# google/deepconsensus

Measured on AMD Instinct MI355X. Metric: zmw_per_sec, higher is better.
Workload: dtype bf16; 1 GPU; global_batch=16384, seq_len=100, windows_per_zmw=150, parallelism=dp1, native_kernels=True, hipgraph=True

## Files before the change

### deepconsensus_amd/models/runner.py

```python
from __future__ import annotations

import copy
import math
from typing import List, Optional, Tuple

import torch

from deepconsensus_amd import ops as dc_ops
from deepconsensus_amd.calibration.calibration import (
    parse_calibration_string,
)
from deepconsensus_amd.models.config import Params
from deepconsensus_amd.models.model import (
    EncoderOnlyLearnedValuesTransformer,
    get_model,
)
from deepconsensus_amd.utils import constants
from deepconsensus_amd.utils import trace


def build_gather_tables(model: EncoderOnlyLearnedValuesTransformer):
    (bi, pwi, ipi, sti, ci, bqi, sni) = model.indices

    def scaled(emb):
# ... 144 lines not shown
            self._prepare_native(model)

    def _prepare_native(self, model) -> None:
        dev, bf16 = self.device, torch.bfloat16
        tf, rs, rv, cc, ce = build_gather_tables(model)
        self.table_flat = tf.to(dev)
        self.row_shift = rs.to(dev)
        self.row_vocab = rv.to(dev)
        self.chunk_cnt = cc.to(dev)
        self.chunk_entries = ce.to(dev)
        self.win = model.params.get("attn_win_size")
        self.num_heads = model.params["num_heads"]
        self.cond_wt = (
            model.condenser.weight.detach().t().contiguous().to(bf16).to(dev)
        )
        self.pos = (
            model.pos_encoding.to(bf16).to(dev)
            if model.add_pos_encoding
            else None
        )
        import os as _os

        self.cond_img = None
        self.pos_f32 = None
        cw = model.condenser.weight.detach()
        if fused_condense_enabled(
            cw.shape[1], _os.environ.get("DC_FUSED_CONDENSE")
        ):
            self.cond_img = build_condense_image(cw).to(dev)
            if model.add_pos_encoding:
                self.pos_f32 = (
                    model.pos_encoding.detach().float().contiguous().to(dev)
                )
        self.rezero_fast = all(
            l.attn_wrap.rezero and l.ffn_wrap.rezero for l in model.layers
        ) and self.win is not None
        if self.rezero_fast:
            self.layer_w = []
            for l in model.layers:
                wq = l.attn.q_proj.weight.detach()
                wk = l.attn.k_proj.weight.detach()
                wv = l.attn.v_proj.weight.detach()
                wqkv_t = (
                    torch.cat([wq, wk, wv], 0).t().contiguous().to(bf16).to(dev)
                )
                self.layer_w.append(
                    dict(
                        wqkv_t=wqkv_t,
                        wout_t=l.attn.out_proj.weight.detach()
                        .t().contiguous().to(bf16).to(dev),
                        w1_t=l.ffn.filter_layer.weight.detach()
                        .t().contiguous().to(bf16).to(dev),
                        b1=l.ffn.filter_layer.bias.detach().to(bf16).to(dev),
                        w2_t=l.ffn.output_layer.weight.detach()
                        .t().contiguous().to(bf16).to(dev),
                        b2=l.ffn.output_layer.bias.detach().to(bf16).to(dev),
                        alpha_attn=float(l.attn_wrap.alpha.detach()),
                        alpha_ffn=float(l.ffn_wrap.alpha.detach()),
                    )
                )
            for lw in self.layer_w:
                lw["wout_t_a"] = lw["wout_t"] * lw["alpha_attn"]
                lw["w2_t_a"] = lw["w2_t"] * lw["alpha_ffn"]
                lw["b2_a"] = lw["b2"] * lw["alpha_ffn"]
            import os as _os

# ... 40 lines not shown
                    lw["w1_v2"] = w1v2.to(bf16).contiguous().to(dev)
            self._addmm_act = hasattr(torch, "_addmm_activation")
            if self._addmm_act:
                try:
                    torch._addmm_activation(
                        torch.zeros(4, device=dev, dtype=bf16),
                        torch.zeros(2, 4, device=dev, dtype=bf16),
                        torch.zeros(4, 4, device=dev, dtype=bf16),
                    )
                except Exception:
                    self._addmm_act = False
        else:
            layers = copy.deepcopy(model.layers).to(bf16)
            for m in layers.modules():
                if isinstance(m, torch.nn.LayerNorm):
                    m.float()
            self.layers_bf16 = layers.to(dev)
        self.ln_gamma = model.output_norm.weight.detach().float().to(dev)
        self.ln_beta = model.output_norm.bias.detach().float().to(dev)
        self.w_head = model.fc1.weight.detach().float().contiguous().to(dev)
        self.b_head = model.fc1.bias.detach().float().to(dev)

    def _attn(self, qkv: torch.Tensor) -> torch.Tensor:
        b, l, w = qkv.shape
        d = w // (3 * self.num_heads)
        if d == 140 and 32 <= l <= 104 and 1 <= self.win <= 12:
            return self.ext.banded_attn_mfma(
                qkv, self.num_heads, self.win, d ** -0.5
            )
        return self.ext.banded_attn(qkv, self.num_heads, self.win)

    @torch.no_grad()
    def encode_native(self, rows: torch.Tensor) -> torch.Tensor:
        with trace.range("K2_embed_gather"):
            emb = self.ext.embed_gather(
                rows.contiguous(), self.table_flat, self.row_shift,
                self.row_vocab, self.chunk_cnt, self.chunk_entries,
            )
        b, l, _ = emb.shape
        if self.cond_img is not None:
            with trace.range("K3_condenser"):
                h = self.cond_wt.shape[1]
                pos = (
                    self.pos_f32
                    if self.pos_f32 is not None
                    else emb.new_empty(0, dtype=torch.float32)
                )
                x = self.ext.fused_condense(
                    emb.reshape(b * l, -1), self.cond_img, pos, h, l
                )
            x = x.view(b, l, -1)
        else:
            with trace.range("K3_condenser"):
                x = emb.reshape(b * l, -1) @ self.cond_wt
            x = x.view(b, l, -1)
            if self.pos is not None:
                x = x + self.pos[:l]
        if self.rezero_fast:
            h = x.shape[-1]
            flat = x.reshape(b * l, h)
            empty = flat.new_empty(0)
            for lw in self.layer_w:
                with trace.range("K5_qkv_proj"):
                    if self.ffn_fused_ok:
                        qkv = self.ext.fused_linear(
                            flat, lw["wqkv_pad"], empty, empty, 840,
                            False, 0.0
                        ).view(b, l, -1)
                    else:
                        qkv = (flat @ lw["wqkv_t"]).view(b, l, -1)
                with trace.range("K6_banded_attn"):
                    a = self._attn(qkv)
                if self.ffn_fused_ok:
                    with trace.range("K7_out_proj"):
                        flat = self.ext.fused_linear(
                            a.view(b * l, h), lw["wout_pad"], empty, flat,
                            280, False, lw["alpha_attn"],
                        )
                    with trace.range("K9_fused_ffn"):
                        if self.ffn_v5:
                            flat = self.ext.fused_ffn_v5(
                                flat, lw["w1_v2"], lw["w2_pad"],
                                lw["b2_f32"], lw["alpha_ffn"],
                            )
                        elif self.ffn_v3:
# ... 109 lines not shown
```

### deepconsensus_amd/ops/build.py

```python
from __future__ import annotations

import os
import shutil

_OPS_DIR = os.path.dirname(os.path.abspath(__file__))
_BUILD_DIR = os.path.join(_OPS_DIR, "_build")
_SRCS = [
    os.path.join(_OPS_DIR, "hip", "dc_kernels.hip"),
    os.path.join(_OPS_DIR, "hip", "banded_attn.hip"),
    os.path.join(_OPS_DIR, "hip", "banded_attn_mfma.hip"),
    os.path.join(_OPS_DIR, "hip", "embed_gather.hip"),
    os.path.join(_OPS_DIR, "hip", "fused_ffn.hip"),
    os.path.join(_OPS_DIR, "hip", "alignment_dp.hip"),
    os.path.join(_OPS_DIR, "hip", "fused_linear.hip"),
    os.path.join(_OPS_DIR, "hip", "fused_ffn_glds.hip"),
    os.path.join(_OPS_DIR, "hip", "fused_ffn_v3.hip"),
    os.path.join(_OPS_DIR, "hip", "embed_grad.hip"),
    os.path.join(_OPS_DIR, "hip", "alignment_metric.hip"),
    os.path.join(_OPS_DIR, "hip", "ffn_ablate.hip"),
    os.path.join(_OPS_DIR, "hip", "banded_attn_train.hip"),
    os.path.join(_OPS_DIR, "hip", "banded_attn_bwd_mfma.hip"),
    os.path.join(_OPS_DIR, "hip", "fused_condense.hip"),
    os.path.join(_OPS_DIR, "hip", "ffn_train.hip"),
    os.path.join(_OPS_DIR, "hip", "resid_dropout.hip"),
    os.path.join(_OPS_DIR, "hip", "stitch_compact.hip"),
    os.path.join(_OPS_DIR, "hip", "window_featurize.hip"),
    os.path.join(_OPS_DIR, "hip", "passthrough_fill.hip"),
    os.path.join(_OPS_DIR, "hip", "subread_space.hip"),
    os.path.join(_OPS_DIR, "hip", "fused_ffn_v5.hip"),
    os.path.join(_OPS_DIR, "hip", "alignment_calib.hip"),
]
EXT_NAME = "dc_hip_kernels"


_SPACING_SRC = os.path.join(
    os.path.dirname(_OPS_DIR), "preprocess", "_spacing_cpp.cpp"
)


def build_spacing(verbose: bool = False):
    os.makedirs(_BUILD_DIR, exist_ok=True)
    from torch.utils.cpp_extension import load

    return load(
        name="_spacing",
        sources=[_SPACING_SRC],
        build_directory=_BUILD_DIR,
        extra_cflags=["-O3"],
        verbose=verbose,
    )


def build(verbose: bool = False):
    os.environ.setdefault("PYTORCH_ROCM_ARCH", "gfx950")
    os.makedirs(_BUILD_DIR, exist_ok=True)
# ... 40 lines not shown
```

### deepconsensus_amd/ops/hip/dc_kernels.hip

```cpp

#ifndef DC_SAN_MAIN
#include <torch/extension.h>
#include <ATen/hip/HIPContext.h>
#endif
#include <hip/hip_runtime.h>
#include <hip/hip_bf16.h>

#define DC_CHECK(x, msg) TORCH_CHECK(x, msg)

using bf16 = __hip_bfloat16;

namespace {

template <typename T>
__global__ __launch_bounds__(256) void fused_ln_head_qv_kernel(
    const T* __restrict__ x, const float* __restrict__ gamma,
    const float* __restrict__ beta, const float* __restrict__ w_head,
    const float* __restrict__ b_head, uint8_t* __restrict__ bases_out,
    uint8_t* __restrict__ quals_out, float* __restrict__ probs_out,
    int N, int H, float cal_threshold, float cal_w, float cal_b,
    float max_qual) {
  const int wave_in_block = threadIdx.x >> 6;
  const int lane = threadIdx.x & 63;
  for (int n = blockIdx.x * 4 + wave_in_block; n < N; n += gridDim.x * 4) {
  const T* xi = x + (size_t)n * H;

  float sum = 0.f;
  float xv[8];
  int nd = 0;
  for (int d = lane; d < H; d += 64, ++nd) {
    float v;
    if constexpr (std::is_same_v<T, bf16>) v = __bfloat162float(xi[d]);
    else v = xi[d];
    xv[nd] = v;
    sum += v;
  }
#pragma unroll
  for (int off = 32; off > 0; off >>= 1) sum += __shfl_xor(sum, off, 64);
  const float mean = sum / H;
  float sq = 0.f;
  nd = 0;
  for (int d = lane; d < H; d += 64, ++nd) {
    const float dv = xv[nd] - mean;
    sq += dv * dv;
  }
#pragma unroll
  for (int off = 32; off > 0; off >>= 1) sq += __shfl_xor(sq, off, 64);
  const float var = sq / H;
  const float rstd = rsqrtf(var + 1e-6f);

  float logit[5];
#pragma unroll
  for (int k = 0; k < 5; ++k) logit[k] = 0.f;
  nd = 0;
  for (int d = lane; d < H; d += 64, ++nd) {
    const float normed = (xv[nd] - mean) * rstd * gamma[d] + beta[d];
#pragma unroll
    for (int k = 0; k < 5; ++k) logit[k] += normed * w_head[k * H + d];
  }
#pragma unroll
  for (int off = 32; off > 0; off >>= 1) {
#pragma unroll
    for (int k = 0; k < 5; ++k) logit[k] += __shfl_xor(logit[k], off, 64);
  }

  if (lane == 0) {
    float mx = -1e30f;
#pragma unroll
    for (int k = 0; k < 5; ++k) {
      logit[k] += b_head[k];
      mx = fmaxf(mx, logit[k]);
    }
    float denom = 0.f;
    float ex[5];
#pragma unroll
    for (int k = 0; k < 5; ++k) {
      ex[k] = __expf(logit[k] - mx);
      denom += ex[k];
    }
    int arg = 0;
    float pmax = 0.f;
#pragma unroll
    for (int k = 0; k < 5; ++k) {
      const float p = ex[k] / denom;
      if (probs_out != nullptr) probs_out[(size_t)n * 5 + k] = p;
      if (p > pmax) { pmax = p; arg = k; }
    }
    float ep = 1.f - pmax;
    float q = (ep <= 0.f) ? 1e9f : -10.f * log10f(ep);
    if (cal_threshold == 0.f || q > cal_threshold) q = q * cal_w + cal_b;
    q = fminf(q, max_qual);
// ... 2 lines not shown
    bases_out[n] = (uint8_t)arg;
    quals_out[n] = (uint8_t)q;
  }
  }
}

}

#ifndef DC_SAN_MAIN

std::vector<at::Tensor> fused_ln_head_qv(
    at::Tensor x, at::Tensor gamma, at::Tensor beta, at::Tensor w_head,
    at::Tensor b_head, double cal_threshold, double cal_w, double cal_b,
    double max_qual, bool want_probs) {
  DC_CHECK(x.is_cuda() && x.dim() >= 2, "x must be a device matrix");
  auto xc = x.contiguous();
  const int H = xc.size(-1);
  const int N = xc.numel() / H;
  DC_CHECK(H <= 512, "H must be <= 512");
  auto opts = xc.options();
  auto bases = at::empty({N}, opts.dtype(at::kByte));
  auto quals = at::empty({N}, opts.dtype(at::kByte));
  at::Tensor probs;
  float* probs_ptr = nullptr;
  if (want_probs) {
    probs = at::empty({N, 5}, opts.dtype(at::kFloat));
    probs_ptr = probs.data_ptr<float>();
  }
  dim3 grid(std::min((N + 3) / 4, 2048));
  dim3 block(256);
  hipStream_t stream = at::hip::getCurrentHIPStream();
  auto gc = gamma.contiguous(), bc = beta.contiguous();
  auto wc = w_head.contiguous(), bhc = b_head.contiguous();
  if (xc.dtype() == at::kBFloat16) {
    hipLaunchKernelGGL(fused_ln_head_qv_kernel<bf16>, grid, block, 0, stream,
                       reinterpret_cast<bf16*>(xc.data_ptr()),
                       gc.data_ptr<float>(), bc.data_ptr<float>(),
                       wc.data_ptr<float>(), bhc.data_ptr<float>(),
                       bases.data_ptr<uint8_t>(), quals.data_ptr<uint8_t>(),
                       probs_ptr, N, H, (float)cal_threshold, (float)cal_w,
                       (float)cal_b, (float)max_qual);
  } else {
    DC_CHECK(xc.dtype() == at::kFloat, "x must be bf16 or fp32");
    hipLaunchKernelGGL(fused_ln_head_qv_kernel<float>, grid, block, 0, stream,
                       xc.data_ptr<float>(), gc.data_ptr<float>(),
                       bc.data_ptr<float>(), wc.data_ptr<float>(),
                       bhc.data_ptr<float>(), bases.data_ptr<uint8_t>(),
                       quals.data_ptr<uint8_t>(), probs_ptr, N, H,
                       (float)cal_threshold, (float)cal_w, (float)cal_b,
                       (float)max_qual);
  }
  if (want_probs) return {bases, quals, probs};
  return {bases, quals};
}

at::Tensor banded_attn(at::Tensor qkv, int64_t H, int64_t win);
at::Tensor banded_attn_mfma(at::Tensor qkv, int64_t H, int64_t win,
                            double scale);
at::Tensor embed_gather(at::Tensor rows, at::Tensor table_flat,
                        at::Tensor row_shift, at::Tensor row_vocab,
                        at::Tensor chunk_cnt, at::Tensor chunk_entries);
at::Tensor fused_ffn(at::Tensor x, at::Tensor w1, at::Tensor b1,
                     at::Tensor w2, at::Tensor b2, double alpha);
at::Tensor fused_ffn_v2(at::Tensor x, at::Tensor w1, at::Tensor w2,
                        at::Tensor b2, double alpha);
at::Tensor fused_ffn_v3(at::Tensor x, at::Tensor w1, at::Tensor w2,
                        at::Tensor b2, double alpha);
at::Tensor fused_ffn_v5(at::Tensor x, at::Tensor w1, at::Tensor w2,
                        at::Tensor b2, double alpha, int64_t max_blocks);
void embed_grad(at::Tensor rows, at::Tensor grad_out, at::Tensor row_shift,
                at::Tensor row_vocab, at::Tensor row_tbase,
                at::Tensor row_width, at::Tensor row_col,
                at::Tensor row_scale, at::Tensor grad_tables);
at::Tensor fused_linear(at::Tensor x, at::Tensor w, at::Tensor bias,
                        at::Tensor resid, int64_t n_out, bool relu,
                        double alpha);
std::vector<at::Tensor> alignment_dp_fwd(at::Tensor subs, at::Tensor ins,
                                         at::Tensor seq_lens, double del_cost,
                                         double reg, int64_t width);
std::vector<at::Tensor> alignment_dp_bwd(at::Tensor grad_out,
                                         at::Tensor weights,
                                         at::Tensor seq_lens, int64_t m,
                                         int64_t n, int64_t width);
std::vector<at::Tensor> alignment_metric_counts(
    at::Tensor yt, at::Tensor yp, at::Tensor yt_len, at::Tensor yp_len,
    double ms, double mp, double go, double ge);
std::vector<at::Tensor> alignment_calib(
    at::Tensor label, at::Tensor bases, at::Tensor quals,
    double ms, double mp, double go, double ge);
at::Tensor ffn_ablate(at::Tensor x, at::Tensor w1, at::Tensor w2,
                      at::Tensor b2, double alpha, int64_t mode);
std::vector<at::Tensor> banded_attn_train_fwd(
    at::Tensor q, at::Tensor k, at::Tensor v, at::Tensor mask,
    int64_t win, double p_drop);
std::vector<at::Tensor> banded_attn_train_bwd(
    at::Tensor q, at::Tensor k, at::Tensor v, at::Tensor p,
    at::Tensor mask, at::Tensor dout, int64_t win, double p_drop);
std::vector<at::Tensor> banded_attn_mfma_train_fwd(
    at::Tensor qkv, int64_t H, int64_t win, double scale,
    at::Tensor drop_mask, double p_drop);
at::Tensor banded_attn_train_bwd2(
    at::Tensor qkv, at::Tensor p, at::Tensor mask, at::Tensor dout,
    int64_t H, int64_t win, double p_drop);
at::Tensor banded_attn_bwd_mfma(
    at::Tensor qkv, at::Tensor p, at::Tensor mask, at::Tensor dout,
    int64_t H, int64_t win, double p_drop);
at::Tensor fused_condense(at::Tensor x, at::Tensor w, at::Tensor pos,
                          int64_t n_out, int64_t seq_len);
std::vector<at::Tensor> ffn_train_fwd(at::Tensor x, at::Tensor w1,
                                      at::Tensor w2, at::Tensor b2,
                                      double p_drop, int64_t seed);
std::vector<at::Tensor> ffn_train_dgrad(at::Tensor dy, at::Tensor hd,
                                        at::Tensor w2t, at::Tensor w1t,
                                        double p_drop);
std::vector<at::Tensor> ffn_train_dgrad_nomask(at::Tensor dy, at::Tensor hd,
                                               at::Tensor w2t,
                                               at::Tensor w1t,
                                               double p_drop);
at::Tensor resid_drop_fwd(at::Tensor x, at::Tensor y, double alpha,
                          double p_drop, int64_t seed);
std::vector<at::Tensor> resid_drop_bwd(at::Tensor dout, at::Tensor y,
                                       double alpha, double p_drop,
                                       int64_t seed);
std::vector<at::Tensor> stitch_compact(at::Tensor bases, at::Tensor quals,
                                       at::Tensor seg_off,
                                       at::Tensor seg_len);
int64_t stitch_compact_into(at::Tensor bases, at::Tensor quals,
                            at::Tensor seg_off, at::Tensor seg_len,
                            at::Tensor seq_out, at::Tensor qual_out,
                            at::Tensor seg_kept, at::Tensor out_off);
at::Tensor window_featurize(at::Tensor sub, at::Tensor ccs,
                            at::Tensor ccs_bq, at::Tensor zmw_tab,
                            at::Tensor win_tab, int64_t R, int64_t L,
                            int64_t max_passes, bool use_ccs_bq);
void window_featurize_into(at::Tensor sub, at::Tensor ccs,
                           at::Tensor ccs_bq, at::Tensor zmw_tab,
                           at::Tensor win_tab, at::Tensor out,
                           int64_t max_passes, bool use_ccs_bq);
void passthrough_fill_into(at::Tensor ccs, at::Tensor ccs_q,
                           at::Tensor zmw_tab, at::Tensor pt_tab,
                           at::Tensor qual_lut, at::Tensor bases_out,
                           at::Tensor quals_out);
void subread_space_into(at::Tensor src, at::Tensor ins_max,
                        at::Tensor sp_tab, at::Tensor read_tab,
                        at::Tensor zmw_tab, at::Tensor col_ref,
                        at::Tensor sub, at::Tensor ccs, at::Tensor ccs_q,
                        at::Tensor ccs_bq, bool use_ccs_bq);
int64_t subread_space_tile();

PYBIND11_MODULE(TORCH_EXTENSION_NAME, m) {
  m.def("subread_space_into", &subread_space_into,
        "Device subread spacing: unspaced reads + ins_max -> caller-owned "
        "zero-filled sub / ccs / ccs_q / ccs_bq planes");
  m.def("subread_space_tile", &subread_space_tile,
        "Scan tile (elements) of subread_space_into");
  m.def("passthrough_fill_into", &passthrough_fill_into,
        "Device CCS passthrough: skipped windows of the packed planes -> "
        "caller-owned base-id and QV rows of the stitch buffer");
  m.def("window_featurize", &window_featurize,
        "Device window featurization: compact ZMW planes + window table "
        "-> int16 [N, R, L] model input");
  m.def("window_featurize_into", &window_featurize_into,
        "window_featurize into a caller-owned int16 [N, R, L] tensor");
  m.def("stitch_compact", &stitch_compact,
        "Device window stitching: segmented gap compaction -> (seq_out, "
        "qual_out, seg_kept, out_off)");
  m.def("stitch_compact_into", &stitch_compact_into,
        "stitch_compact into caller-owned output buffers; returns "
        "out_off[S]");
  m.def("fused_condense", &fused_condense,
        "Condenser GEMM [M,560]x[560,N] + fused position-encoding add "
        "(K3+K4)");
  m.def("ffn_train_fwd", &ffn_train_fwd,
        "Training FFN forward: relu + hash dropout in-register, returns "
        "(y, hd)");
  m.def("ffn_train_dgrad", &ffn_train_dgrad,
        "Training FFN dgrad: both transposed GEMMs fused, mask from hd>0, "
        "returns (dx, dh_pre)");
  m.def("ffn_train_dgrad_nomask", &ffn_train_dgrad_nomask,
        "Bisection probe: dgrad without the mask (dh == dy@W2^T)");
  m.def("resid_drop_fwd", &resid_drop_fwd,
        "Fused ReZero residual + hash-dropout forward");
  m.def("resid_drop_bwd", &resid_drop_bwd,
        "Fused residual-dropout backward: (dy, dalpha partials)");
  m.def("fused_ln_head_qv", &fused_ln_head_qv,
        "Fused final LayerNorm + head + softmax + QV (K10+K11+K12)");
  m.def("banded_attn", &banded_attn,
        "Banded multi-head self-attention forward (K5-K7 core, generic)");
  m.def("banded_attn_mfma", &banded_attn_mfma,
        "Banded MHA forward on MFMA (D=140, L<=104)");
  m.def("embed_gather", &embed_gather,
        "Subread-stack embedding gather (K2)");
  m.def("fused_ffn", &fused_ffn,
        "Fused FFN + ReZero residual (K8+K9), hidden tensor LDS-resident");
  m.def("fused_ffn_v2", &fused_ffn_v2,
        "Fused FFN v2: glds-pipelined weights, bias folded into W1");
  m.def("fused_ffn_v3", &fused_ffn_v3,
        "Fused FFN v3: 256-row tiles, register-resident h (swapped B1)");
  m.def("fused_ffn_v5", &fused_ffn_v5,
        "Fused FFN v5: v3 chunk loop in a persistent grid (continuous "
        "weight stream, direct x fragments, 16-B epilogue); max_blocks "
        "caps the grid, 0 = one block per CU",
        pybind11::arg("x"), pybind11::arg("w1"), pybind11::arg("w2"),
        pybind11::arg("b2"), pybind11::arg("alpha"),
        pybind11::arg("max_blocks") = 0);
// ... 33 lines not shown
```

### deepconsensus_amd/ops/hip/fused_condense.hip

```cpp

#ifndef DC_SAN_MAIN
#include <torch/extension.h>
#include <ATen/hip/HIPContext.h>
#endif
#include <hip/hip_runtime.h>
#include <hip/hip_bf16.h>

using bf16 = __hip_bfloat16;

namespace {

typedef __bf16 bf16x8 __attribute__((ext_vector_type(8)));
typedef float f32x16 __attribute__((ext_vector_type(16)));

constexpr int NC = 64;
constexpr int O_STRIDE = 72;

template <int K>
struct CondCfg {
  static constexpr int NG = (K + 15) / 16;
  static constexpr int WS = 16 * NG + 8;
  static constexpr bool HALF = (K % 16) == 8;
  static constexpr int NW = NG <= 36 ? 8 : 4;
  static constexpr int BM = 32 * NW;
  static constexpr int NT = 64 * NW;
  static constexpr int UNITS = NC * WS * 2 / 1024;
  static_assert(K % 8 == 0, "rows must stay 16-B aligned");
  static_assert((NC * WS * 2) % 1024 == 0, "chunk must be whole KiB units");
  static_assert((NC * WS + BM * O_STRIDE) * 2 <= 160 * 1024, "LDS budget");
};

__device__ __forceinline__ int lane_recompute() {
  int l;
  asm volatile(
      "v_mbcnt_lo_u32_b32 %0, -1, 0\n\t"
      "v_mbcnt_hi_u32_b32 %0, -1, %0"
      : "=v"(l));
  return l;
}

template <int K>
__global__ __launch_bounds__(CondCfg<K>::NT, 1) void fused_condense_kernel(
    const bf16* __restrict__ x, const bf16* __restrict__ w,
    const float* __restrict__ pos, bf16* __restrict__ out,
    int M, int N, int Npad, int L) {
  using C = CondCfg<K>;
  constexpr int NG = C::NG;
  constexpr int W_STRIDE = C::WS;
  constexpr int BM = C::BM;
  constexpr int NW = C::NW;
  constexpr int NT = C::NT;
  __shared__ __attribute__((aligned(16))) bf16 w_lds[NC * W_STRIDE];
  __shared__ __attribute__((aligned(16))) bf16 o_lds[BM * O_STRIDE];

  const int tid = threadIdx.x;
  const int wave = __builtin_amdgcn_readfirstlane(tid >> 6);
  const int m0 = blockIdx.x * BM;

  auto issue_w = [&](int chunk) {
    const int ln = lane_recompute();
    const bf16* src = w + (size_t)chunk * NC * W_STRIDE;
    constexpr int TRIPS = (C::UNITS + NW - 1) / NW;
    constexpr int UNROLL = NW == 8 ? TRIPS : 4;
#pragma unroll UNROLL
    for (int i = 0; i < TRIPS; ++i) {
      const int ck = wave + i * NW;
      if (ck < C::UNITS) {
        __builtin_amdgcn_global_load_lds(
            (const __attribute__((address_space(1))) unsigned*)(
                src + ck * 512 + ln * 8),
            (__attribute__((address_space(3))) unsigned*)(
                &w_lds[ck * 512]),
            16, 0, 0);
      }
    }
  };

  issue_w(0);

  bf16x8 af[NG];
  {
    const int ln = lane_recompute();
    const int row = m0 + 32 * wave + (ln & 31);
    constexpr int NFULL = C::HALF ? NG - 1 : NG;
    if (row < M) {
      const bf16* xr = x + (size_t)row * K + 8 * (ln >> 5);
#pragma unroll
      for (int s = 0; s < NFULL; ++s) {
        af[s] = *reinterpret_cast<const bf16x8*>(xr + 16 * s);
      }
    } else {
#pragma unroll
      for (int s = 0; s < NFULL; ++s) af[s] = bf16x8{};
    }
    if constexpr (C::HALF) {
      af[NG - 1] = bf16x8{};
      if (row < M && (ln >> 5) == 0) {
        af[NG - 1] = *reinterpret_cast<const bf16x8*>(
            x + (size_t)row * K + 16 * (NG - 1));
      }
    }
  }
  asm volatile("s_waitcnt vmcnt(0)" ::: "memory");
  __builtin_amdgcn_s_barrier();

  const int nchunk = Npad / NC;
  for (int chunk = 0; chunk < nchunk; ++chunk) {
    const int ln = lane_recompute();
    const int c = ln & 31;
    const int hi = ln >> 5;
#pragma unroll
    for (int ch = 0; ch < 2; ++ch) {
      const int colt = 32 * ch;
      const int ncol = chunk * NC + colt + c;
      f32x16 acc0 = {}, acc1 = {};
      __builtin_amdgcn_s_setprio(1);
#pragma unroll
      for (int s = 0; s < NG; s += 2) {
        const bf16x8 b0 = *reinterpret_cast<const bf16x8*>(
            &w_lds[(colt + c) * W_STRIDE + 16 * s + 8 * hi]);
        acc0 = __builtin_amdgcn_mfma_f32_32x32x16_bf16(af[s], b0, acc0,
                                                       0, 0, 0);
        if (s + 1 < NG) {
          const bf16x8 b1 = *reinterpret_cast<const bf16x8*>(
              &w_lds[(colt + c) * W_STRIDE + 16 * (s + 1) + 8 * hi]);
          acc1 = __builtin_amdgcn_mfma_f32_32x32x16_bf16(af[s + 1], b1,
                                                         acc1, 0, 0, 0);
        }
      }
      __builtin_amdgcn_s_setprio(0);
#pragma unroll
      for (int r = 0; r < 16; ++r) {
        const int row = (r & 3) + 8 * (r >> 2) + 4 * hi + 32 * wave;
        float v = acc0[r] + acc1[r];
        if (pos != nullptr && ncol < N && m0 + row < M) {
          v += pos[(size_t)((m0 + row) % L) * N + ncol];
        }
        o_lds[row * O_STRIDE + colt + c] = __float2bfloat16(v);
      }
    }
    __syncthreads();
    if (chunk + 1 < nchunk) issue_w(chunk + 1);

    const int n0 = chunk * NC;
    for (int idx = tid; idx < BM * (NC / 8); idx += NT) {
      const int row = idx / (NC / 8), c8 = idx % (NC / 8);
      if (m0 + row >= M) continue;
      const int col = n0 + 8 * c8;
      if (col >= N) continue;
      const bf16x8 v = *reinterpret_cast<const bf16x8*>(
          &o_lds[row * O_STRIDE + 8 * c8]);
      if (col + 8 <= N) {
        *reinterpret_cast<bf16x8*>(
            out + (size_t)(m0 + row) * N + col) = v;
      } else {
        const unsigned short* vs =
            reinterpret_cast<const unsigned short*>(&v);
        for (int j = 0; j < 8 && col + j < N; ++j) {
          reinterpret_cast<unsigned short*>(
              out)[(size_t)(m0 + row) * N + col + j] = vs[j];
        }
      }
    }
    if (chunk + 1 < nchunk) {
      asm volatile("s_waitcnt vmcnt(0) lgkmcnt(0)" ::: "memory");
    }
    __builtin_amdgcn_s_barrier();
  }
}

#define DC_CONDENSE_INST(K)                                       \
  template __global__ void fused_condense_kernel<K>(              \
      const bf16* __restrict__, const bf16* __restrict__,         \
      const float* __restrict__, bf16* __restrict__, int, int, int, int)
DC_CONDENSE_INST(560);
DC_CONDENSE_INST(568);
DC_CONDENSE_INST(872);
DC_CONDENSE_INST(880);
#undef DC_CONDENSE_INST

}

#ifndef DC_SAN_MAIN

namespace {

template <int K>
void launch_condense(const at::Tensor& xc, const at::Tensor& w,
                     const float* pos_ptr, at::Tensor& out, int M, int N,
                     int Npad, int L) {
  using C = CondCfg<K>;
  TORCH_CHECK(w.size(1) == C::WS, "fused_condense: width-", K,
              " input needs a weight image of row stride ", C::WS,
              ", got ", w.size(1));
  dim3 grid((M + C::BM - 1) / C::BM);
  dim3 block(C::NT);
  hipStream_t stream = at::hip::getCurrentHIPStream();
  hipLaunchKernelGGL(fused_condense_kernel<K>, grid, block, 0, stream,
                     reinterpret_cast<bf16*>(xc.data_ptr()),
                     reinterpret_cast<bf16*>(w.data_ptr()), pos_ptr,
                     reinterpret_cast<bf16*>(out.data_ptr()), M, N, Npad,
// ... 44 lines not shown
```

Before: 2471 ZMWs/sec.

## Fuse embedding gather into condenser GEMM and register-cache LN head params

Adds a fused kernel that gathers embedding rows directly into MFMA A-fragments inside the condenser GEMM, so the intermediate [M,K] embedding tensor is never written to or read back from global memory. The shared condense tile code moves into a header and both kernels use it. The LN+head kernel also keeps gamma, beta and the head weights in registers and prefetches the next row. The cost is more register pressure and scattered gathers inside the GEMM prologue.

```diff
diff --git a/deepconsensus_amd/models/runner.py b/deepconsensus_amd/models/runner.py
--- a/deepconsensus_amd/models/runner.py
+++ b/deepconsensus_amd/models/runner.py
@@ -200,6 +200,7 @@
                 self.pos_f32 = (
                     model.pos_encoding.detach().float().contiguous().to(dev)
                 )
+        self.fused_embed = _os.environ.get("DC_FUSED_EMBED") != "0"
         self.rezero_fast = all(
             l.attn_wrap.rezero and l.ffn_wrap.rezero for l in model.layers
         ) and self.win is not None
@@ -306,25 +307,35 @@
 
     @torch.no_grad()
     def encode_native(self, rows: torch.Tensor) -> torch.Tensor:
-        with trace.range("K2_embed_gather"):
-            emb = self.ext.embed_gather(
-                rows.contiguous(), self.table_flat, self.row_shift,
-                self.row_vocab, self.chunk_cnt, self.chunk_entries,
-            )
-        b, l, _ = emb.shape
+        rows = rows.contiguous()
+        b, _, l = rows.shape
+        gather_args = (
+            rows, self.table_flat, self.row_shift, self.row_vocab,
+            self.chunk_cnt, self.chunk_entries,
+        )
         if self.cond_img is not None:
-            with trace.range("K3_condenser"):
-                h = self.cond_wt.shape[1]
-                pos = (
-                    self.pos_f32
-                    if self.pos_f32 is not None
-                    else emb.new_empty(0, dtype=torch.float32)
-                )
-                x = self.ext.fused_condense(
-                    emb.reshape(b * l, -1), self.cond_img, pos, h, l
-                )
+            h = self.cond_wt.shape[1]
+            pos = (
+                self.pos_f32
+                if self.pos_f32 is not None
+                else torch.empty(0, dtype=torch.float32, device=rows.device)
+            )
+            if self.fused_embed:
+                with trace.range("K2_K3_embed_condense"):
+                    x = self.ext.fused_embed_condense(
+                        *gather_args, self.cond_img, pos, h
+                    )
+            else:
+                with trace.range("K2_embed_gather"):
+                    emb = self.ext.embed_gather(*gather_args)
+                with trace.range("K3_condenser"):
+                    x = self.ext.fused_condense(
+                        emb.reshape(b * l, -1), self.cond_img, pos, h, l
+                    )
             x = x.view(b, l, -1)
         else:
+            with trace.range("K2_embed_gather"):
+                emb = self.ext.embed_gather(*gather_args)
             with trace.range("K3_condenser"):
                 x = emb.reshape(b * l, -1) @ self.cond_wt
             x = x.view(b, l, -1)
diff --git a/deepconsensus_amd/ops/build.py b/deepconsensus_amd/ops/build.py
--- a/deepconsensus_amd/ops/build.py
+++ b/deepconsensus_amd/ops/build.py
@@ -21,6 +21,7 @@
     os.path.join(_OPS_DIR, "hip", "banded_attn_train.hip"),
     os.path.join(_OPS_DIR, "hip", "banded_attn_bwd_mfma.hip"),
     os.path.join(_OPS_DIR, "hip", "fused_condense.hip"),
+    os.path.join(_OPS_DIR, "hip", "fused_embed_condense.hip"),
     os.path.join(_OPS_DIR, "hip", "ffn_train.hip"),
     os.path.join(_OPS_DIR, "hip", "resid_dropout.hip"),
     os.path.join(_OPS_DIR, "hip", "stitch_compact.hip"),
diff --git a/deepconsensus_amd/ops/hip/condense_tile.h b/deepconsensus_amd/ops/hip/condense_tile.h
--- /dev/null
+++ b/deepconsensus_amd/ops/hip/condense_tile.h
@@ -0,0 +1,144 @@
+#pragma once
+
+#include <hip/hip_runtime.h>
+#include <hip/hip_bf16.h>
+
+using bf16 = __hip_bfloat16;
+
+namespace {
+
+typedef __bf16 bf16x8 __attribute__((ext_vector_type(8)));
+typedef float f32x16 __attribute__((ext_vector_type(16)));
+
+constexpr int NC = 64;
+constexpr int O_STRIDE = 72;
+
+template <int K>
+struct CondCfg {
+  static constexpr int NG = (K + 15) / 16;
+  static constexpr int WS = 16 * NG + 8;
+  static constexpr bool HALF = (K % 16) == 8;
+  static constexpr int NW = NG <= 36 ? 8 : 4;
+  static constexpr int BM = 32 * NW;
+  static constexpr int NT = 64 * NW;
+  static constexpr int UNITS = NC * WS * 2 / 1024;
+  static_assert(K % 8 == 0, "rows must stay 16-B aligned");
+  static_assert((NC * WS * 2) % 1024 == 0, "chunk must be whole KiB units");
+  static_assert((NC * WS + BM * O_STRIDE) * 2 <= 160 * 1024, "LDS budget");
+};
+
+__device__ __forceinline__ int lane_recompute() {
+  int l;
+  asm volatile(
+      "v_mbcnt_lo_u32_b32 %0, -1, 0\n\t"
+      "v_mbcnt_hi_u32_b32 %0, -1, %0"
+      : "=v"(l));
+  return l;
+}
+
+template <int K>
+__device__ __forceinline__ void cond_issue_w(
+    const bf16* __restrict__ w, bf16 (&w_lds)[NC * CondCfg<K>::WS], int wave,
+    int chunk) {
+  using C = CondCfg<K>;
+  constexpr int NW = C::NW;
+  const int ln = lane_recompute();
+  const bf16* src = w + (size_t)chunk * NC * C::WS;
+  constexpr int TRIPS = (C::UNITS + NW - 1) / NW;
+  constexpr int UNROLL = NW == 8 ? TRIPS : 4;
+#pragma unroll UNROLL
+  for (int i = 0; i < TRIPS; ++i) {
+    const int ck = wave + i * NW;
+    if (ck < C::UNITS) {
+      __builtin_amdgcn_global_load_lds(
+          (const __attribute__((address_space(1))) unsigned*)(
+              src + ck * 512 + ln * 8),
+          (__attribute__((address_space(3))) unsigned*)(
+              &w_lds[ck * 512]),
+          16, 0, 0);
+    }
+  }
+}
+
+template <int K>
+__device__ __forceinline__ void cond_chunk_loop(
+    const bf16x8 (&af)[CondCfg<K>::NG], const bf16* __restrict__ w,
+    const float* __restrict__ pos, bf16* __restrict__ out,
+    bf16 (&w_lds)[NC * CondCfg<K>::WS],
+    bf16 (&o_lds)[CondCfg<K>::BM * O_STRIDE], int M, int N, int Npad, int L,
+    int tid, int wave, int m0) {
+  using C = CondCfg<K>;
+  constexpr int NG = C::NG;
+  constexpr int W_STRIDE = C::WS;
+  constexpr int BM = C::BM;
+  constexpr int NT = C::NT;
+
+  asm volatile("s_waitcnt vmcnt(0)" ::: "memory");
+  __builtin_amdgcn_s_barrier();
+
+  const int nchunk = Npad / NC;
+  for (int chunk = 0; chunk < nchunk; ++chunk) {
+    const int ln = lane_recompute();
+    const int c = ln & 31;
+    const int hi = ln >> 5;
+#pragma unroll
+    for (int ch = 0; ch < 2; ++ch) {
+      const int colt = 32 * ch;
+      const int ncol = chunk * NC + colt + c;
+      f32x16 acc0 = {}, acc1 = {};
+      __builtin_amdgcn_s_setprio(1);
+#pragma unroll
+      for (int s = 0; s < NG; s += 2) {
+        const bf16x8 b0 = *reinterpret_cast<const bf16x8*>(
+            &w_lds[(colt + c) * W_STRIDE + 16 * s + 8 * hi]);
+        acc0 = __builtin_amdgcn_mfma_f32_32x32x16_bf16(af[s], b0, acc0,
+                                                       0, 0, 0);
+        if (s + 1 < NG) {
+          const bf16x8 b1 = *reinterpret_cast<const bf16x8*>(
+              &w_lds[(colt + c) * W_STRIDE + 16 * (s + 1) + 8 * hi]);
+          acc1 = __builtin_amdgcn_mfma_f32_32x32x16_bf16(af[s + 1], b1,
+                                                         acc1, 0, 0, 0);
+        }
+      }
+      __builtin_amdgcn_s_setprio(0);
+#pragma unroll
+      for (int r = 0; r < 16; ++r) {
+        const int row = (r & 3) + 8 * (r >> 2) + 4 * hi + 32 * wave;
+        float v = acc0[r] + acc1[r];
+        if (pos != nullptr && ncol < N && m0 + row < M) {
+          v += pos[(size_t)((m0 + row) % L) * N + ncol];
+        }
+        o_lds[row * O_STRIDE + colt + c] = __float2bfloat16(v);
+      }
+    }
+    __syncthreads();
+    if (chunk + 1 < nchunk) cond_issue_w<K>(w, w_lds, wave, chunk + 1);
+
+    const int n0 = chunk * NC;
+    for (int idx = tid; idx < BM * (NC / 8); idx += NT) {
+      const int row = idx / (NC / 8), c8 = idx % (NC / 8);
+      if (m0 + row >= M) continue;
+      const int col = n0 + 8 * c8;
+      if (col >= N) continue;
+      const bf16x8 v = *reinterpret_cast<const bf16x8*>(
+          &o_lds[row * O_STRIDE + 8 * c8]);
+      if (col + 8 <= N) {
+        *reinterpret_cast<bf16x8*>(
+            out + (size_t)(m0 + row) * N + col) = v;
+      } else {
+        const unsigned short* vs =
+            reinterpret_cast<const unsigned short*>(&v);
+        for (int j = 0; j < 8 && col + j < N; ++j) {
+          reinterpret_cast<unsigned short*>(
+              out)[(size_t)(m0 + row) * N + col + j] = vs[j];
+        }
+      }
+    }
+    if (chunk + 1 < nchunk) {
+      asm volatile("s_waitcnt vmcnt(0) lgkmcnt(0)" ::: "memory");
+    }
+    __builtin_amdgcn_s_barrier();
+  }
+}
+
+}
diff --git a/deepconsensus_amd/ops/hip/dc_kernels.hip b/deepconsensus_amd/ops/hip/dc_kernels.hip
--- a/deepconsensus_amd/ops/hip/dc_kernels.hip
+++ b/deepconsensus_amd/ops/hip/dc_kernels.hip
@@ -12,7 +12,7 @@
 
 namespace {
 
-template <typename T>
+template <typename T, int NS = 8>
 __global__ __launch_bounds__(256) void fused_ln_head_qv_kernel(
     const T* __restrict__ x, const float* __restrict__ gamma,
     const float* __restrict__ beta, const float* __restrict__ w_head,
@@ -22,27 +22,65 @@
     float max_qual) {
   const int wave_in_block = threadIdx.x >> 6;
   const int lane = threadIdx.x & 63;
-  for (int n = blockIdx.x * 4 + wave_in_block; n < N; n += gridDim.x * 4) {
-  const T* xi = x + (size_t)n * H;
-
+
+  float g[NS], bt[NS], wh[5][NS];
+#pragma unroll
+  for (int j = 0; j < NS; ++j) {
+    const int d = lane + 64 * j;
+    g[j] = 0.f;
+    bt[j] = 0.f;
+#pragma unroll
+    for (int k = 0; k < 5; ++k) wh[k][j] = 0.f;
+    if (d < H) {
+      g[j] = gamma[d];
+      bt[j] = beta[d];
+#pragma unroll
+      for (int k = 0; k < 5; ++k) wh[k][j] = w_head[k * H + d];
+    }
+  }
+
+  const int stride = gridDim.x * 4;
+  int n = blockIdx.x * 4 + wave_in_block;
+  T xr[NS];
+  if (n < N) {
+    const T* xi = x + (size_t)n * H;
+#pragma unroll
+    for (int j = 0; j < NS; ++j) {
+      const int d = lane + 64 * j;
+      if (d < H) xr[j] = xi[d];
+    }
+  }
+  for (; n < N; n += stride) {
   float sum = 0.f;
-  float xv[8];
-  int nd = 0;
-  for (int d = lane; d < H; d += 64, ++nd) {
-    float v;
-    if constexpr (std::is_same_v<T, bf16>) v = __bfloat162float(xi[d]);
-    else v = xi[d];
-    xv[nd] = v;
-    sum += v;
+  float xv[NS];
+#pragma unroll
+  for (int j = 0; j < NS; ++j) {
+    if (lane + 64 * j < H) {
+      float v;
+      if constexpr (std::is_same_v<T, bf16>) v = __bfloat162float(xr[j]);
+      else v = xr[j];
+      xv[j] = v;
+      sum += v;
+    }
+  }
+  if (n + stride < N) {
+    const T* xi = x + (size_t)(n + stride) * H;
+#pragma unroll
+    for (int j = 0; j < NS; ++j) {
+      const int d = lane + 64 * j;
+      if (d < H) xr[j] = xi[d];
+    }
   }
 #pragma unroll
   for (int off = 32; off > 0; off >>= 1) sum += __shfl_xor(sum, off, 64);
   const float mean = sum / H;
   float sq = 0.f;
-  nd = 0;
-  for (int d = lane; d < H; d += 64, ++nd) {
-    const float dv = xv[nd] - mean;
-    sq += dv * dv;
+#pragma unroll
+  for (int j = 0; j < NS; ++j) {
+    if (lane + 64 * j < H) {
+      const float dv = xv[j] - mean;
+      sq += dv * dv;
+    }
   }
 #pragma unroll
   for (int off = 32; off > 0; off >>= 1) sq += __shfl_xor(sq, off, 64);
@@ -52,11 +90,13 @@
   float logit[5];
 #pragma unroll
   for (int k = 0; k < 5; ++k) logit[k] = 0.f;
-  nd = 0;
-  for (int d = lane; d < H; d += 64, ++nd) {
-    const float normed = (xv[nd] - mean) * rstd * gamma[d] + beta[d];
-#pragma unroll
-    for (int k = 0; k < 5; ++k) logit[k] += normed * w_head[k * H + d];
+#pragma unroll
+  for (int j = 0; j < NS; ++j) {
+    if (lane + 64 * j < H) {
+      const float normed = (xv[j] - mean) * rstd * g[j] + bt[j];
+#pragma unroll
+      for (int k = 0; k < 5; ++k) logit[k] += normed * wh[k][j];
+    }
   }
 #pragma unroll
   for (int off = 32; off > 0; off >>= 1) {
@@ -125,23 +165,26 @@
   hipStream_t stream = at::hip::getCurrentHIPStream();
   auto gc = gamma.contiguous(), bc = beta.contiguous();
   auto wc = w_head.contiguous(), bhc = b_head.contiguous();
+  auto launch = [&](auto tag) {
+    using T = decltype(tag);
+    auto go = [&](auto kern) {
+      hipLaunchKernelGGL(kern, grid, block, 0, stream,
+                         reinterpret_cast<const T*>(xc.data_ptr()),
+                         gc.data_ptr<float>(), bc.data_ptr<float>(),
+                         wc.data_ptr<float>(), bhc.data_ptr<float>(),
+                         bases.data_ptr<uint8_t>(), quals.data_ptr<uint8_t>(),
+                         probs_ptr, N, H, (float)cal_threshold, (float)cal_w,
+                         (float)cal_b, (float)max_qual);
+    };
+    if (H <= 128) go(fused_ln_head_qv_kernel<T, 2>);
+    else if (H <= 320) go(fused_ln_head_qv_kernel<T, 5>);
+    else go(fused_ln_head_qv_kernel<T, 8>);
+  };
   if (xc.dtype() == at::kBFloat16) {
-    hipLaunchKernelGGL(fused_ln_head_qv_kernel<bf16>, grid, block, 0, stream,
-                       reinterpret_cast<bf16*>(xc.data_ptr()),
-                       gc.data_ptr<float>(), bc.data_ptr<float>(),
-                       wc.data_ptr<float>(), bhc.data_ptr<float>(),
-                       bases.data_ptr<uint8_t>(), quals.data_ptr<uint8_t>(),
-                       probs_ptr, N, H, (float)cal_threshold, (float)cal_w,
-                       (float)cal_b, (float)max_qual);
+    launch(bf16{});
   } else {
     DC_CHECK(xc.dtype() == at::kFloat, "x must be bf16 or fp32");
-    hipLaunchKernelGGL(fused_ln_head_qv_kernel<float>, grid, block, 0, stream,
-                       xc.data_ptr<float>(), gc.data_ptr<float>(),
-                       bc.data_ptr<float>(), wc.data_ptr<float>(),
-                       bhc.data_ptr<float>(), bases.data_ptr<uint8_t>(),
-                       quals.data_ptr<uint8_t>(), probs_ptr, N, H,
-                       (float)cal_threshold, (float)cal_w, (float)cal_b,
-                       (float)max_qual);
+    launch(float{});
   }
   if (want_probs) return {bases, quals, probs};
   return {bases, quals};
@@ -200,6 +243,11 @@
     int64_t H, int64_t win, double p_drop);
 at::Tensor fused_condense(at::Tensor x, at::Tensor w, at::Tensor pos,
                           int64_t n_out, int64_t seq_len);
+at::Tensor fused_embed_condense(at::Tensor rows, at::Tensor table_flat,
+                                at::Tensor row_shift, at::Tensor row_vocab,
+                                at::Tensor chunk_cnt,
+                                at::Tensor chunk_entries, at::Tensor w,
+                                at::Tensor pos, int64_t n_out);
 std::vector<at::Tensor> ffn_train_fwd(at::Tensor x, at::Tensor w1,
                                       at::Tensor w2, at::Tensor b2,
                                       double p_drop, int64_t seed);
@@ -264,6 +312,9 @@
   m.def("fused_condense", &fused_condense,
         "Condenser GEMM [M,560]x[560,N] + fused position-encoding add "
         "(K3+K4)");
+  m.def("fused_embed_condense", &fused_embed_condense,
+        "Embedding gather inside the condenser GEMM + position-encoding "
+        "add (K2+K3+K4): fused_condense(embed_gather(rows)) bit for bit");
   m.def("ffn_train_fwd", &ffn_train_fwd,
         "Training FFN forward: relu + hash dropout in-register, returns "
         "(y, hd)");
diff --git a/deepconsensus_amd/ops/hip/fused_condense.hip b/deepconsensus_amd/ops/hip/fused_condense.hip
--- a/deepconsensus_amd/ops/hip/fused_condense.hip
+++ b/deepconsensus_amd/ops/hip/fused_condense.hip
@@ -6,38 +6,9 @@
 #include <hip/hip_runtime.h>
 #include <hip/hip_bf16.h>
 
-using bf16 = __hip_bfloat16;
+#include "condense_tile.h"
 
 namespace {
-
-typedef __bf16 bf16x8 __attribute__((ext_vector_type(8)));
-typedef float f32x16 __attribute__((ext_vector_type(16)));
-
-constexpr int NC = 64;
-constexpr int O_STRIDE = 72;
-
-template <int K>
-struct CondCfg {
-  static constexpr int NG = (K + 15) / 16;
-  static constexpr int WS = 16 * NG + 8;
-  static constexpr bool HALF = (K % 16) == 8;
-  static constexpr int NW = NG <= 36 ? 8 : 4;
-  static constexpr int BM = 32 * NW;
-  static constexpr int NT = 64 * NW;
-  static constexpr int UNITS = NC * WS * 2 / 1024;
-  static_assert(K % 8 == 0, "rows must stay 16-B aligned");
-  static_assert((NC * WS * 2) % 1024 == 0, "chunk must be whole KiB units");
-  static_assert((NC * WS + BM * O_STRIDE) * 2 <= 160 * 1024, "LDS budget");
-};
-
-__device__ __forceinline__ int lane_recompute() {
-  int l;
-  asm volatile(
-      "v_mbcnt_lo_u32_b32 %0, -1, 0\n\t"
-      "v_mbcnt_hi_u32_b32 %0, -1, %0"
-      : "=v"(l));
-  return l;
-}
 
 template <int K>
 __global__ __launch_bounds__(CondCfg<K>::NT, 1) void fused_condense_kernel(
@@ -48,8 +19,6 @@
   constexpr int NG = C::NG;
   constexpr int W_STRIDE = C::WS;
   constexpr int BM = C::BM;
-  constexpr int NW = C::NW;
-  constexpr int NT = C::NT;
   __shared__ __attribute__((aligned(16))) bf16 w_lds[NC * W_STRIDE];
   __shared__ __attribute__((aligned(16))) bf16 o_lds[BM * O_STRIDE];
 
@@ -57,26 +26,7 @@
   const int wave = __builtin_amdgcn_readfirstlane(tid >> 6);
   const int m0 = blockIdx.x * BM;
 
-  auto issue_w = [&](int chunk) {
-    const int ln = lane_recompute();
-    const bf16* src = w + (size_t)chunk * NC * W_STRIDE;
-    constexpr int TRIPS = (C::UNITS + NW - 1) / NW;
-    constexpr int UNROLL = NW == 8 ? TRIPS : 4;
-#pragma unroll UNROLL
-    for (int i = 0; i < TRIPS; ++i) {
-      const int ck = wave + i * NW;
-      if (ck < C::UNITS) {
-        __builtin_amdgcn_global_load_lds(
-            (const __attribute__((address_space(1))) unsigned*)(
-                src + ck * 512 + ln * 8),
-            (__attribute__((address_space(3))) unsigned*)(
-                &w_lds[ck * 512]),
-            16, 0, 0);
-      }
-    }
-  };
-
-  issue_w(0);
+  cond_issue_w<K>(w, w_lds, wave, 0);
 
   bf16x8 af[NG];
   {
@@ -101,72 +51,8 @@
       }
     }
   }
-  asm volatile("s_waitcnt vmcnt(0)" ::: "memory");
-  __builtin_amdgcn_s_barrier();
-
-  const int nchunk = Npad / NC;
-  for (int chunk = 0; chunk < nchunk; ++chunk) {
-    const int ln = lane_recompute();
-    const int c = ln & 31;
-    const int hi = ln >> 5;
-#pragma unroll
-    for (int ch = 0; ch < 2; ++ch) {
-      const int colt = 32 * ch;
-      const int ncol = chunk * NC + colt + c;
-      f32x16 acc0 = {}, acc1 = {};
-      __builtin_amdgcn_s_setprio(1);
-#pragma unroll
-      for (int s = 0; s < NG; s += 2) {
-        const bf16x8 b0 = *reinterpret_cast<const bf16x8*>(
-            &w_lds[(colt + c) * W_STRIDE + 16 * s + 8 * hi]);
-        acc0 = __builtin_amdgcn_mfma_f32_32x32x16_bf16(af[s], b0, acc0,
-                                                       0, 0, 0);
-        if (s + 1 < NG) {
-          const bf16x8 b1 = *reinterpret_cast<const bf16x8*>(
-              &w_lds[(colt + c) * W_STRIDE + 16 * (s + 1) + 8 * hi]);
-          acc1 = __builtin_amdgcn_mfma_f32_32x32x16_bf16(af[s + 1], b1,
-                                                         acc1, 0, 0, 0);
-        }
-      }
-      __builtin_amdgcn_s_setprio(0);
-#pragma unroll
-      for (int r = 0; r < 16; ++r) {
-        const int row = (r & 3) + 8 * (r >> 2) + 4 * hi + 32 * wave;
-        float v = acc0[r] + acc1[r];
-        if (pos != nullptr && ncol < N && m0 + row < M) {
-          v += pos[(size_t)((m0 + row) % L) * N + ncol];
-        }
-        o_lds[row * O_STRIDE + colt + c] = __float2bfloat16(v);
-      }
-    }
-    __syncthreads();
-    if (chunk + 1 < nchunk) issue_w(chunk + 1);
-
-    const int n0 = chunk * NC;
-    for (int idx = tid; idx < BM * (NC / 8); idx += NT) {
-      const int row = idx / (NC / 8), c8 = idx % (NC / 8);
-      if (m0 + row >= M) continue;
-      const int col = n0 + 8 * c8;
-      if (col >= N) continue;
-      const bf16x8 v = *reinterpret_cast<const bf16x8*>(
-          &o_lds[row * O_STRIDE + 8 * c8]);
-      if (col + 8 <= N) {
-        *reinterpret_cast<bf16x8*>(
-            out + (size_t)(m0 + row) * N + col) = v;
-      } else {
-        const unsigned short* vs =
-            reinterpret_cast<const unsigned short*>(&v);
-        for (int j = 0; j < 8 && col + j < N; ++j) {
-          reinterpret_cast<unsigned short*>(
-              out)[(size_t)(m0 + row) * N + col + j] = vs[j];
-        }
-      }
-    }
-    if (chunk + 1 < nchunk) {
-      asm volatile("s_waitcnt vmcnt(0) lgkmcnt(0)" ::: "memory");
-    }
-    __builtin_amdgcn_s_barrier();
-  }
+  cond_chunk_loop<K>(af, w, pos, out, w_lds, o_lds, M, N, Npad, L, tid, wave,
+                     m0);
 }
 
 #define DC_CONDENSE_INST(K)                                       \
diff --git a/deepconsensus_amd/ops/hip/fused_embed_condense.hip b/deepconsensus_amd/ops/hip/fused_embed_condense.hip
--- /dev/null
+++ b/deepconsensus_amd/ops/hip/fused_embed_condense.hip
@@ -0,0 +1,246 @@
+
+#ifndef DC_SAN_MAIN
+#include <torch/extension.h>
+#include <ATen/hip/HIPContext.h>
+#endif
+#include <hip/hip_runtime.h>
+#include <hip/hip_bf16.h>
+
+#include "condense_tile.h"
+
+namespace {
+
+constexpr int MAX_R = 160;
+
+template <typename TIn>
+__device__ __forceinline__ int cond_row_id(const TIn* __restrict__ rp,
+                                           size_t off, int shift,
+                                           int vocab) {
+  const int id = (int)rp[off] + shift;
+  const int vmax = vocab - 1;
+  return (short)(id < 0 ? 0 : (id > vmax ? vmax : id));
+}
+
+template <typename TIn>
+__device__ __forceinline__ bf16x8 cond_gather_chunk(
+    const TIn* __restrict__ rp, const bf16* __restrict__ table_flat,
+    const int* __restrict__ row_shift, const int* __restrict__ row_vocab,
+    const int4* __restrict__ chunk_entries, int c, int cnt, int L) {
+  uint4 raw;
+  if (cnt == 1) {
+    const int4 e = chunk_entries[c * 4];
+    const int id = cond_row_id(rp, (size_t)e.x * L, row_shift[e.x],
+                               row_vocab[e.x]);
+    raw = *reinterpret_cast<const uint4*>(table_flat + e.y + (size_t)id * 8);
+  } else {
+    unsigned d[4] = {0u, 0u, 0u, 0u};
+#pragma unroll
+    for (int k = 0; k < 4; ++k) {
+      if (k < cnt) {
+        const int4 e = chunk_entries[c * 4 + k];
+        const int id = cond_row_id(rp, (size_t)e.x * L, row_shift[e.x],
+                                   row_vocab[e.x]);
+        d[k] = *reinterpret_cast<const unsigned*>(
+            table_flat + e.y + (size_t)id * 2);
+      }
+    }
+    raw.x = d[0];
+    raw.y = d[1];
+    raw.z = d[2];
+    raw.w = d[3];
+  }
+  return __builtin_bit_cast(bf16x8, raw);
+}
+
+template <int K, typename TIn>
+__global__ __launch_bounds__(CondCfg<K>::NT, 1)
+void fused_embed_condense_kernel(
+    const TIn* __restrict__ rows,
+    const bf16* __restrict__ table_flat,
+    const int* __restrict__ row_shift,
+    const int* __restrict__ row_vocab,
+    const int* __restrict__ chunk_cnt,
+    const int4* __restrict__ chunk_entries,
+    const bf16* __restrict__ w, const float* __restrict__ pos,
+    bf16* __restrict__ out, int M, int N, int Npad, int R, int L) {
+  using C = CondCfg<K>;
+  constexpr int NG = C::NG;
+  constexpr int BM = C::BM;
+  __shared__ __attribute__((aligned(16))) bf16 w_lds[NC * C::WS];
+  __shared__ __attribute__((aligned(16))) bf16 o_lds[BM * O_STRIDE];
+
+  const int tid = threadIdx.x;
+  const int wave = __builtin_amdgcn_readfirstlane(tid >> 6);
+  const int m0 = blockIdx.x * BM;
+
+  cond_issue_w<K>(w, w_lds, wave, 0);
+
+  bf16x8 af[NG];
+  {
+    const int ln = lane_recompute();
+    const int row = m0 + 32 * wave + (ln & 31);
+    const int hi = ln >> 5;
+    constexpr int NFULL = C::HALF ? NG - 1 : NG;
+    if (row < M) {
+      const int b = row / L;
+      const TIn* rp = rows + (size_t)b * R * L + (row - b * L);
+#pragma unroll
+      for (int s = 0; s < NFULL; ++s) {
+        const int cnt0 = chunk_cnt[2 * s], cnt1 = chunk_cnt[2 * s + 1];
+        if (cnt0 == 1 && cnt1 == 1) {
+          const int4 e0 = chunk_entries[8 * s];
+          const int4 e1 = chunk_entries[8 * s + 4];
+          const int sh0 = row_shift[e0.x], sh1 = row_shift[e1.x];
+          const int vc0 = row_vocab[e0.x], vc1 = row_vocab[e1.x];
+          const size_t o0 = (size_t)e0.x * L, o1 = (size_t)e1.x * L;
+          const int id = cond_row_id(rp, hi ? o1 : o0, hi ? sh1 : sh0,
+                                     hi ? vc1 : vc0);
+          af[s] = *reinterpret_cast<const bf16x8*>(
+              table_flat + (hi ? e1.y : e0.y) + (size_t)id * 8);
+        } else {
+          af[s] = cond_gather_chunk(rp, table_flat, row_shift, row_vocab,
+                                    chunk_entries, 2 * s + hi,
+                                    hi ? cnt1 : cnt0, L);
+        }
+      }
+      if constexpr (C::HALF) {
+        af[NG - 1] = bf16x8{};
+        if (hi == 0) {
+          af[NG - 1] = cond_gather_chunk(
+              rp, table_flat, row_shift, row_vocab, chunk_entries,
+              2 * (NG - 1), chunk_cnt[2 * (NG - 1)], L);
+        }
+      }
+    } else {
+#pragma unroll
+      for (int s = 0; s < NG; ++s) af[s] = bf16x8{};
+    }
+  }
+  cond_chunk_loop<K>(af, w, pos, out, w_lds, o_lds, M, N, Npad, L, tid, wave,
+                     m0);
+}
+
+#define DC_EMBED_CONDENSE_INST(K, T)                                       \
+  template __global__ void fused_embed_condense_kernel<K, T>(              \
+      const T* __restrict__, const bf16* __restrict__,                     \
+      const int* __restrict__, const int* __restrict__,                    \
+      const int* __restrict__, const int4* __restrict__,                   \
+      const bf16* __restrict__, const float* __restrict__,                 \
+      bf16* __restrict__, int, int, int, int, int)
+DC_EMBED_CONDENSE_INST(560, short);
+DC_EMBED_CONDENSE_INST(568, short);
+DC_EMBED_CONDENSE_INST(872, short);
+DC_EMBED_CONDENSE_INST(880, short);
+DC_EMBED_CONDENSE_INST(560, float);
+DC_EMBED_CONDENSE_INST(568, float);
+DC_EMBED_CONDENSE_INST(872, float);
+DC_EMBED_CONDENSE_INST(880, float);
+#undef DC_EMBED_CONDENSE_INST
+
+}
+
+#ifndef DC_SAN_MAIN
+
+namespace {
+
+template <int K, typename TIn>
+void launch_embed_condense(const at::Tensor& rc, const at::Tensor& table_flat,
+                           const at::Tensor& row_shift,
+                           const at::Tensor& row_vocab,
+                           const at::Tensor& chunk_cnt,
+                           const at::Tensor& chunk_entries,
+                           const at::Tensor& w, const float* pos_ptr,
+                           at::Tensor& out, int M, int N, int Npad, int R,
+                           int L) {
+  using C = CondCfg<K>;
+  TORCH_CHECK(w.size(1) == C::WS, "fused_embed_condense: width-", K,
+              " input needs a weight image of row stride ", C::WS,
+              ", got ", w.size(1));
+  dim3 grid((M + C::BM - 1) / C::BM);
+  dim3 block(C::NT);
+  hipStream_t stream = at::hip::getCurrentHIPStream();
+  hipLaunchKernelGGL((fused_embed_condense_kernel<K, TIn>), grid, block, 0,
+                     stream, rc.data_ptr<TIn>(),
+                     reinterpret_cast<bf16*>(table_flat.data_ptr()),
+                     row_shift.data_ptr<int>(), row_vocab.data_ptr<int>(),
+                     chunk_cnt.data_ptr<int>(),
+                     reinterpret_cast<int4*>(chunk_entries.data_ptr<int>()),
+                     reinterpret_cast<bf16*>(w.data_ptr()), pos_ptr,
+                     reinterpret_cast<bf16*>(out.data_ptr()), M, N, Npad, R,
+                     L);
+}
+
+template <typename TIn, typename... Args>
+void dispatch_embed_condense(int K, Args&&... args) {
+  switch (K) {
+    case 560: launch_embed_condense<560, TIn>(args...); break;
+    case 568: launch_embed_condense<568, TIn>(args...); break;
+    case 872: launch_embed_condense<872, TIn>(args...); break;
+    default:  launch_embed_condense<880, TIn>(args...); break;
+  }
+}
+
+}
+
+at::Tensor fused_embed_condense(
+    at::Tensor rows, at::Tensor table_flat, at::Tensor row_shift,
+    at::Tensor row_vocab, at::Tensor chunk_cnt, at::Tensor chunk_entries,
+    at::Tensor w, at::Tensor pos, int64_t n_out) {
+  TORCH_CHECK(rows.is_cuda() && rows.dim() == 3 &&
+                  (rows.dtype() == at::kFloat || rows.dtype() == at::kShort),
+              "rows must be float32 or int16 [B, R, L] on device");
+  TORCH_CHECK(table_flat.is_cuda() && table_flat.is_contiguous() &&
+                  table_flat.dtype() == at::kBFloat16,
+              "tables must be contiguous bf16 on device");
+  auto rc = rows.contiguous();
+  const int B = rc.size(0), R = rc.size(1), L = rc.size(2);
+  TORCH_CHECK(R <= MAX_R, "too many rows");
+  auto is_map = [](const at::Tensor& t) {
+    return t.is_cuda() && t.is_contiguous() && t.dtype() == at::kInt;
+  };
+  TORCH_CHECK(is_map(row_shift) && is_map(row_vocab) && is_map(chunk_cnt) &&
+                  is_map(chunk_entries),
+              "gather map tensors must be contiguous int32 on device");
+  TORCH_CHECK(row_shift.numel() == R && row_vocab.numel() == R,
+              "row_shift / row_vocab must have one entry per input row (", R,
+              ")");
+  const int nchunk = chunk_cnt.numel();
+  const int K = 8 * nchunk;
+  TORCH_CHECK(K == 560 || K == 568 || K == 872 || K == 880,
+              "fused_embed_condense requires concat width 560, 568, 872 or "
+              "880, got ", K);
+  TORCH_CHECK(chunk_entries.numel() == (int64_t)nchunk * 16,
+              "chunk_entries must hold 4 x int4 per chunk");
+  TORCH_CHECK(w.is_cuda() && w.dim() == 2 && w.is_contiguous() &&
+                  w.dtype() == at::kBFloat16 && w.size(0) % NC == 0,
+              "w must be contiguous bf16 [Npad (mult of 64), WS] on device");
+  const int Npad = w.size(0);
+  const int N = (int)n_out;
+  TORCH_CHECK(N <= Npad, "n_out exceeds padded weight rows");
+  const int64_t M64 = (int64_t)B * L;
+  TORCH_CHECK(M64 < (1LL << 31) - 256, "too many positions");
+  const int M = (int)M64;
+  const float* pos_ptr = nullptr;
+  at::Tensor pc;
+  if (pos.defined() && pos.numel() > 0) {
+    pc = pos.contiguous();
+    TORCH_CHECK(pc.is_cuda() && pc.dtype() == at::kFloat &&
+                    pc.size(-1) == N && pc.numel() >= (int64_t)L * N,
+                "pos must be fp32 [>=L, N] on device");
+    pos_ptr = pc.data_ptr<float>();
+  }
+  auto out = at::empty({M, N}, rc.options().dtype(at::kBFloat16));
+  if (M == 0) return out;
+  if (rc.dtype() == at::kFloat) {
+    dispatch_embed_condense<float>(K, rc, table_flat, row_shift, row_vocab,
+                                   chunk_cnt, chunk_entries, w, pos_ptr, out,
+                                   M, N, Npad, R, L);
+  } else {
+    dispatch_embed_condense<short>(K, rc, table_flat, row_shift, row_vocab,
+                                   chunk_cnt, chunk_entries, w, pos_ptr, out,
+                                   M, N, Npad, R, L);
+  }
+  return out;
+}
+
+#endif
```

After: 2561 ZMWs/sec (median of 6 runs). 3.6% higher.
